# google-research/FirstOrderLp.jl

Measured on AMD Instinct MI355X. Metric: pdhg_iterations_per_sec, higher is better.
Workload: dtype f64; 1 GPU; random LP m=10000000 n=10000000 nnz=100000000 seed=12345 (BASELINE configs[4]), adaptive step, zero start, no restarts/rescaling; id=configs[4], m=10000000, n=10000000, nnz=100000000, parallelism=single GPU

## Files before the change

firstorderlp.jl_amd/csrc/abi_measure.hpp:

```cpp


int pdhg_profile_enable(pdhg_handle *h, int enable) {
  int rc0 = check_handle(h);
  if (rc0) return rc0;
  h->profile = enable != 0;
  if (enable) for (int k = 0; k < PDHG_K_COUNT; ++k) { h->prof_count[k] = 0; h->prof_ms[k] = 0.0; }
  return 0;
}

int pdhg_profile_read(pdhg_handle *h, int kernel_id, int64_t *launches, double *total_ms) {
  if (!h || kernel_id < 0 || kernel_id >= PDHG_K_COUNT) return fail(-1, "bad kernel id");
  *launches = h->prof_count[kernel_id];
  *total_ms = h->prof_ms[kernel_id];
  return 0;
}

int64_t pdhg_kernel_algorithmic_bytes(pdhg_handle *h, int kernel_id) {
  if (!h) return -1;
  const int64_t m = h->m, n = h->n, nnz = h->nnz, cn = h->cn;
  const bool group = h->grp != nullptr;
  switch (kernel_id) {
    case PDHG_K_PRIMAL: return 8 * (7 + (h->lazy_accept ? 2 : 0)) * cn;
    case PDHG_K_SPMV_DUAL:
      return nnz * 12 + (m + 1) * 4 + n * 8 + (3 + (h->lazy_accept ? 2 : 0)) * m * 8;
    case PDHG_K_SPMV_ATY:
      return nnz * 12 + (n + 1) * 4 + m * 8 + (group ? 1 : 4) * n * 8;
    case PDHG_K_FINAL: return 8 * (int64_t)(3 * h->At.slots() + h->A.slots());
    case PDHG_K_ACCEPT: return 8 * 3 * (cn + m);
    case PDHG_K_ALLGATHER: return group ? 8 * (h->n_alloc - h->grp->S) : 0;
    case PDHG_K_REDUCE_SCATTER: return group ? 8 * (h->n_alloc - h->grp->S) : 0;
    case PDHG_K_INTERACTION: return group ? 8 * 4 * cn : 0;
    default: return -1;
  }
}

namespace {
typedef double dbl2_t __attribute__((ext_vector_type(2)));
__global__ __launch_bounds__(TPB) void triad_kernel(int64_t len4, const dbl2_t *__restrict__ b,
                                                    const dbl2_t *__restrict__ c, double s,
                                                    dbl2_t *__restrict__ a) {
  const int64_t stride = (int64_t)gridDim.x * TPB;
  for (int64_t i = (int64_t)blockIdx.x * TPB + threadIdx.x; i < len4; i += stride) {
    const int64_t k = 2 * i;
    const dbl2_t b0 = __builtin_nontemporal_load(b + k), b1 = __builtin_nontemporal_load(b + k + 1);
    const dbl2_t c0 = __builtin_nontemporal_load(c + k), c1 = __builtin_nontemporal_load(c + k + 1);
// ... 288 lines not shown
    snprintf(b, sizeof b, ", \"sliced_jagged\": {\"window_rows\": %d, \"slices_per_wave\": %d, \"hub_threshold\": %d, \"hub_rows\": %lld, \"hub_nnz\": %lld, "
             "\"fill_narrow\": %.3f, \"fill_wide\": %.3f, \"ragged_share\": %.3f, \"grid\": %d}", SJ_SIGMA * J->G, J->G, J->max_len, (long long)hub, (long long)hub_nnz,
             J->fill_narrow, J->fill_wide, J->ragged, J->grid);
    out += b;
  }
  return out + "}";
}

int pdhg_layout_describe(pdhg_handle *h, char *buf, int cap) {
  if (!h) return fail(-1, "null handle");
  std::string out = "{\"A\": " + describe_matrix(h, h->A, MODE_DUAL, 0) + ", \"At\": " + describe_matrix(h, h->At, h->grp ? MODE_PLAIN : MODE_ATY, 1);
  if (h->has_q) out += ", \"Q\": " + describe_matrix(h, h->Q, MODE_PLAIN, 2) + ", \"Qt\": " + describe_matrix(h, h->Qt, MODE_PLAIN, 2);
  if (h->grp && !h->Achunk.empty()) {
    char b[256];
    snprintf(b, sizeof b, ", \"all_gather\": {\"chunks\": %d, \"mode\": \"%s\", \"columns_per_rank_and_chunk\": %lld, \"passes\": [",
             (int)h->Achunk.size(), (h->grp->ag_mode == 1 && h->grp->backend == COMM_RCCL) ? "overlapped with A_p xbar" : "passes behind one all-gather",
             (long long)h->grp->ag_sub);
    out += b;
    for (size_t c = 0; c < h->Achunk.size(); ++c)
      out += (c ? ", " : "") + describe_matrix(h, h->Achunk[c], c + 1 < h->Achunk.size() ? MODE_PLAIN : MODE_DUAL, 0);
    out += "]}";
  }
  const char *tv = getenv("PDHG_TUNE");
  out += std::string(", \"row_order\": \"") + (h->relaxed ? "relaxed" : "strict") + "\", \"timing_at_create\": " + ((tv && tv[0] == '0') ? "false" : "true") + "}";
  if (buf && cap > 0) {
    const size_t k = std::min(out.size(), (size_t)cap - 1);
    memcpy(buf, out.data(), k);
    buf[k] = 0;
  }
  return (int)out.size();
}

int pdhg_layout_info(pdhg_handle *h, int64_t info[16]) {
  if (!h) return fail(-1, "null handle");
  info[12] = (int64_t)h->A.slabs.size(); info[13] = (int64_t)h->At.slabs.size();
  info[14] = (coop_eligible(h) || h->coop_mode == 1) ? 2 : ((graph_eligible(h) || (h->graph_mode == 1 && !h->has_q)) ? 1 : 0);
  info[15] = ((h->A.tiled && h->A.var_tiles) || (!h->A.segs.empty() && h->A.segs.front().tiled && h->A.segs.front().var_tiles) ? 1 : 0) +
             ((h->At.tiled && h->At.var_tiles) || (!h->At.segs.empty() && h->At.segs.front().tiled && h->At.segs.front().var_tiles) ? 2 : 0) +
             (small_lp_eligible(h) ? 4 : 0) +
             (!h->grp && !h->has_q && !small_lp_eligible(h) && device_loop_for(h) && coop_eligible(h) ? 8 : 0) +
             (h->local_mode == 1 && h->local_launches > 0 ? 16 : 0);
  auto total = [](const CsrDev &D, auto f) { int64_t t = 0; if (D.segs.empty()) return (int64_t)f(D); for (const CsrDev &S : D.segs) t += f(S); return t; };
  auto first = [](const CsrDev &D) -> const CsrDev & { return D.segs.empty() ? D : D.segs.front(); };
  const CsrDev *Ms[2] = {&h->A, &h->At};
  for (int k = 0; k < 2; ++k) {
    const CsrDev &D = *Ms[k];
    info[4 * k + 0] = total(D, [](const CsrDev &S) { return S.nblk; });
// ... 21 lines not shown
```

firstorderlp.jl_amd/csrc/abi_rescale.hpp:

```cpp


static int row_grid(int rows) { return std::max(1, (rows + (TPB / WAVE) - 1) / (TPB / WAVE)); }

struct RescaleTmp {
  double *ev = nullptr, *dv = nullptr, *inv_e = nullptr, *inv_d = nullptr, *cum_e = nullptr, *cum_d = nullptr;
  double *tmp_e = nullptr, *tmp_d = nullptr;
};

extern "C++" {
template <int OP>
static void launch_row_op(pdhg_handle *h, const CsrDev &D, int cols, double pexp, const double *inv_scale, double *out) {
  if (!D.segs.empty()) {
    for (const CsrDev &S : D.segs) launch_row_op<OP>(h, S, cols, pexp, inv_scale ? inv_scale + S.row0 : inv_scale, out + S.row0);
    return;
  }
  hipLaunchKernelGGL(row_op_kernel<OP>, dim3(row_grid(D.rows)), dim3(TPB), 0, h->stream, D.view(), cols, pexp, inv_scale, out,
                     D.long_thr);
  if (D.nlong > 0) {
    hipLaunchKernelGGL(row_op_long_partial_kernel<OP>, dim3(D.nchunks), dim3(TPB), 0, h->stream, D.view(),
                       (const int *)D.chunk_row, (const int *)D.chunk_off, pexp, inv_scale, D.chunk_partial);
    hipLaunchKernelGGL(row_op_long_final_kernel<OP>, dim3(D.long_grid), dim3(TPB), 0, h->stream, D.view(),
                       (const int *)D.long_row, (const int *)D.long_chunk_ptr, D.nlong,
                       (const double *)D.chunk_partial, cols, pexp, out);
  }
// ... 23 lines not shown
        hipLaunchKernelGGL(scale_csr_kernel, dim3(row_grid(D.rows)), dim3(TPB), 0, h->stream, D.rows, S.rowptr,
                           S.col, S.val, inv_e, inv_d, k, 0);
    auto refill = [&](const SjDev &J, const int *rowptr, const int *col, const double *val) {
      if (J.on() && J.nnz > 0)
        hipLaunchKernelGGL(sj_fill_kernel, dim3((J.nslices + TPB / WAVE - 1) / (TPB / WAVE)), dim3(TPB), 0, h->stream, J.nslices, (TPB / WAVE) * J.G,
                           (const unsigned *)J.meta, (const int *)J.slice_off, rowptr, col, val, J.col, J.val);
    };
    refill(D.sj, D.rowptr, D.col, D.val);
    for (const SlabDev &S : D.slabs) refill(S.sj, S.rowptr, S.col, S.val);
  };
  scale_one(h->A, t.inv_e, t.inv_d, 0);
  scale_one(h->At, t.inv_e, t.inv_d, 1);
  if (!h->Achunk.empty() && h->grp) {
    DistGroup &g = *h->grp;
    int rc2 = launch_chunk_pack(g, t.inv_d, h->xchunk, 0, g.world, h->n, h->stream);
    if (rc2) return rc2;
    const int64_t W = (int64_t)g.world * g.ag_sub;
    for (size_t c = 0; c < h->Achunk.size(); ++c) scale_one(h->Achunk[c], t.inv_e, h->xchunk + (int64_t)c * W, 0);
  }
  if (h->has_q) {
    scale_one(h->Q, t.inv_d, t.inv_d, 0);
    scale_one(h->Qt, t.inv_d, t.inv_d, 1);
  }
  hipLaunchKernelGGL(resc_apply_vectors_kernel, dim3(h->ew_grid_nm), dim3(TPB), 0, h->stream, n, m, t.dv, t.ev,
                     h->c, h->lb, h->ub, h->b, t.cum_d, t.cum_e);
  HIP_TRY(hipGetLastError());
  if (h->bat) return batch_scale_members(h, t.dv, t.ev);
  return 0;
}

int pdhg_rescale(pdhg_handle *h0, int l_inf_ruiz_iterations, int l2_norm_rescaling,
                 int use_pock_chambolle, double pock_chambolle_alpha,
                 double *constraint_rescaling_out, double *variable_rescaling_out) {
  int rc = check_handle(h0, true, true);
  if (rc) return rc;
  if (h0->owner) return fail(-1, "pdhg_rescale: a batch member shares its batch's matrix: rescale the batch handle");
  if (use_pock_chambolle && !(pock_chambolle_alpha >= 0.0 && pock_chambolle_alpha <= 2.0))
    return fail(-1, "pock_chambolle_alpha must be in [0, 2]");
  const Shards L = shards_of(h0);
  if ((rc = flush_pending(L))) return rc;
  bump_version(L);
  for (int i = 0; i < L.count; ++i) L.p[i]->matrix_version += 1;
  std::vector<RescaleTmp> T((size_t)L.count);
  auto cleanup = [&]() {
    for (int i = 0; i < L.count; ++i) {
      (void)hipSetDevice(L.p[i]->device);
// ... 135 lines not shown
```

firstorderlp.jl_amd/csrc/common.hpp:

```cpp
#pragma once

namespace {

constexpr int TPB = 256;
constexpr int WAVE = 64;
constexpr int BLOCK_NNZ = 2048;
constexpr int UNROLL = BLOCK_NNZ / TPB;
#ifndef PDHG_MAX_ROWS_PER_BLOCK
#define PDHG_MAX_ROWS_PER_BLOCK (4 * TPB)
#endif
constexpr int MAX_ROWS_PER_BLOCK = PDHG_MAX_ROWS_PER_BLOCK;
inline const char *dev_env(const char *name) {
  static const bool on = [] { const char *e = getenv("PDHG_DEV"); return e && e[0] == '1'; }();
  return on ? getenv(name) : nullptr;
}
constexpr int LONG_CHUNK = BLOCK_NNZ;
inline int long_row_threshold_from_env() {
  const char *e = dev_env("PDHG_LONG_THR");
  const int v = e ? atoi(e) : BLOCK_NNZ;
  return v < 16 ? 16 : (v > BLOCK_NNZ ? BLOCK_NNZ : v);
}
constexpr int NUM_XCD = 8;
constexpr int EW_MAX_BLOCKS = 256 * 8;
inline int ew_grid(int64_t len) {
  return (int)std::max<int64_t>(1, std::min<int64_t>((len + TPB - 1) / TPB, EW_MAX_BLOCKS));
}
constexpr int FINAL_TPB = 1024;
constexpr int TW_WPB = 8;
constexpr int TW_MAX_ROWS = 1272;
constexpr unsigned TW_PAD = 0xFFFFFFFFu;
#ifndef TWD_U
#define TWD_U 4
#endif
constexpr int TW_U = TWD_U;

thread_local std::string g_last_error;

int fail(int code, const std::string &msg) {
  g_last_error = msg;
  return code;
}

int fail_hip(hipError_t e, const char *what) {
  g_last_error = std::string(what) + ": " + hipGetErrorString(e);
  return (int)e > 0 ? (int)e : 999;
}

#define HIP_TRY(expr)                                                        \
  do {                                                                       \
    hipError_t _e = (expr);                                                  \
    if (_e != hipSuccess) {                                                  \
      g_last_error = std::string(#expr) + ": " + hipGetErrorString(_e);      \
      return (int)_e > 0 ? (int)_e : 999;                                    \
    }                                                                        \
  } while (0)

struct RoctxApi {
// ... 176 lines not shown
```

firstorderlp.jl_amd/csrc/host_shards.hpp:

```cpp


template <typename Src, typename Dst>
int gather_cols_device(const Shards &L, Src src, Dst dst) {
  if (!L.g) {
    pdhg_handle *s = L.p[0];
    if (src(s) != dst(s))
      HIP_TRY(hipMemcpyAsync(dst(s), src(s), sizeof(double) * (size_t)s->n, hipMemcpyDeviceToDevice, s->stream));
    return 0;
  }
  FOR_SHARDS(L, s) {
    if (src(s) != dst(s) && s->cn > 0)
      HIP_TRY(hipMemcpyAsync(dst(s) + s->clo, src(s) + s->clo, sizeof(double) * (size_t)s->cn,
                             hipMemcpyDeviceToDevice, s->stream));
  }
  return dist_all_gather(*L.g, dst, L.g->S);
}

template <typename Src>
int cols_to_host(const Shards &L, Src src, double *host) {
  if (!L.g || L.g->all_local()) {
    FOR_SHARDS(L, s) {
      if (s->cn > 0)
        HIP_TRY(hipMemcpyAsync(host + s->clo, src(s) + s->clo, sizeof(double) * (size_t)s->cn, hipMemcpyDeviceToHost, s->stream));
    }
// ... 428 lines not shown
    if (len > 0) { HIP_TRY(hipMemcpy(*dst, src, sizeof(double) * (size_t)len, hipMemcpyHostToDevice)); HIP_TRY(hipStreamSynchronize(nullptr)); }
    return 0;
  };
  CK(up(&h->c, c, n)); CK(up(&h->b, b, m)); CK(up(&h->lb, lb, n)); CK(up(&h->ub, ub, n));
  CK(alloc_zero(&h->x, n_alloc)); CK(alloc_zero(&h->x_next, n_alloc)); CK(alloc_zero(&h->xbar, n_alloc));
  CK(alloc_zero(&h->y, m)); CK(alloc_zero(&h->y_next, m));
  CK(alloc_zero(&h->aty, n_alloc + 1)); CK(alloc_zero(&h->aty_next, n_alloc + 1));
  CK(alloc_zero(&h->sum_x, n)); CK(alloc_zero(&h->sum_y, m));
  CK(alloc_zero(&h->tmp_n, n_alloc)); CK(alloc_zero(&h->tmp_m, m));
  h->ew_grid_n = ew_grid(n); h->ew_grid_m = ew_grid(m); h->ew_grid_nm = ew_grid(std::max(n, m));
  h->pAt_stride = std::max(h->At.slots(), h->ew_grid_n);
  CK(alloc_zero(&h->pA, 2 * (int64_t)std::max(h->A.slots(), 1)));
  CK(alloc_zero(&h->pAt, 6 * (int64_t)std::max(h->pAt_stride, 1)));
  CK(alloc_zero(&h->pQ, 2 * (int64_t)h->ew_grid_n));
  CK(alloc_zero(&h->scal_dev, SCAL_MAX));
#undef CK
  hipError_t e = hipHostMalloc((void **)&h->scal_host, sizeof(double) * SCAL_MAX * DIST_MAX_WORLD, hipHostMallocDefault);
  if (e != hipSuccess) return fail((int)e, "hipHostMalloc failed");
  e = hipEventCreate(&h->ev0); if (e == hipSuccess) e = hipEventCreate(&h->ev1);
  if (e != hipSuccess) return fail((int)e, "hipEventCreate failed");
  return 0;
}

int create_shard(pdhg_handle **out, int64_t m, int64_t n, int64_t nnz,
                 const int64_t *colptr, const int64_t *rowval, const double *nzval,
                 int index_base, const double *c, const double *b, const double *lb,
                 const double *ub, int64_t num_equalities, int device_id, void *stream, int64_t n_alloc, int64_t seg_cap) {
  *out = nullptr;
  if (index_base != 0 && index_base != 1) return fail(-1, "index_base must be 0 or 1");
  if (num_equalities < 0 || num_equalities > m) return fail(-1, "num_equalities out of range");
  if (!colptr || !c || !lb || !ub || (m > 0 && !b) || (nnz > 0 && (!rowval || !nzval)))
    return fail(-1, "null input array");
  int ndev = 0;
  HIP_TRY(hipGetDeviceCount(&ndev));
  if (ndev <= 0) return fail(-3, "no HIP device visible");
  int dev = device_id;
  if (dev < 0) HIP_TRY(hipGetDevice(&dev));
  if (dev >= ndev) return fail(-1, "device_id out of range");
  HIP_TRY(hipSetDevice(dev));
  n_alloc = std::max(n_alloc, n);

  pdhg_handle *h = new pdhg_handle();
  h->self = h;
  h->device = dev;
  h->m = m; h->n = n; h->nnz = nnz; h->num_eq = num_equalities;
  h->cn = n; h->n_alloc = n_alloc; h->m_global = m;
  const char *env = getenv("PDHG_XCD_REMAP");
  h->remap = !(env && env[0] == '0');
  env = getenv("PDHG_ROW_ORDER");
  h->relaxed = !(env && !strcmp(env, "strict"));
  env = getenv("PDHG_LAZY_ACCEPT");
  h->lazy_accept = !(env && env[0] == '0');
  if (stream) { h->stream = (hipStream_t)stream; h->own_stream = false; }
  else {
    hipError_t e = hipStreamCreateWithFlags(&h->stream, hipStreamNonBlocking);
    if (e != hipSuccess) { delete h; return fail((int)e, "hipStreamCreate failed"); }
    h->own_stream = true;
  }
#define CK(expr) do { int _rc = (expr); if (_rc) { destroy_shard(h); return _rc; } } while (0)
  if (seg_cap > 0 && nnz > seg_cap) CK(build_segments(dev, h, m, n, nnz, colptr, rowval, nzval, index_base, seg_cap));
  else CK(build_layout_pair(dev, h->remap, h->relaxed, m, n, nnz, colptr, rowval, nzval, index_base, &h->A, &h->At));
  CK(alloc_shard_vectors(h, c, b, lb, ub));
  CK(tune_tiled_variant(h, h->A, h->xbar, h->tmp_m));
  CK(tune_tiled_variant(h, h->At, h->y, h->tmp_n));
#undef CK
  HIP_TRY(hipDeviceSynchronize());
  *out = h;
  return 0;
}

int trial_timeline(pdhg_handle *h, double out[14]) {
  if (!h->coop_trace || h->coop_grid <= 0) return 1;
  std::vector<unsigned long long> t((size_t)8 * h->coop_grid);
  if (hipMemcpy(t.data(), h->coop_trace, sizeof(unsigned long long) * t.size(), hipMemcpyDeviceToHost) != hipSuccess) return 1;
  unsigned long long t0 = ~0ull;
  for (int w = 0; w < h->coop_grid; ++w) t0 = std::min(t0, t[(size_t)w * 8]);
  for (int k = 0; k < 5; ++k) {
    double sum = 0, mx = 0, last_end = 0;
    for (int w = 0; w < h->coop_grid; ++w) {
      const double d = 0.01 * (double)(t[(size_t)w * 8 + k + 1] - t[(size_t)w * 8 + k]);
      sum += d; mx = std::max(mx, d);
      last_end = std::max(last_end, 0.01 * (double)(t[(size_t)w * 8 + k + 1] - t0));
    }
    out[k] = sum / h->coop_grid;
    out[5 + k] = mx;
// ... 24 lines not shown
      for (int k = 0; k < 5; ++k)
        fprintf(stderr, "    %-38s mean %6.2f us, max %6.2f us; last workgroup out at %6.2f us\n", names[k], t[k], t[5 + k], h->timeline_last_out[k]);
      if (t[11] > 0) fprintf(stderr, "    barrier 3: global phase complete at %6.2f us; decision known to the last workgroup at %6.2f us (multi-step kernel, last trial)\n",
                             t[11], t[12]);
      else fprintf(stderr, "    second-stage reduction published at %6.2f us\n", t[12]);
    }
  }
  if (!h->owner) { free_csr_dev(h->A); free_csr_dev(h->At); }
  free_csr_dev(h->Q); free_csr_dev(h->Qt);
  for (CsrDev &D : h->Achunk) free_csr_dev(D);
  if (h->chunk_carry) (void)hipFree(h->chunk_carry);
  if (h->xchunk) (void)hipFree(h->xchunk);
  for (hipEvent_t ev : h->ev_ag) if (ev) (void)hipEventDestroy(ev);
  if (h->ev_xbar) (void)hipEventDestroy(h->ev_xbar);
  double *bufs[] = {h->c, h->b, h->lb, h->ub, h->x, h->x_next, h->xbar, h->y, h->y_next,
                    h->aty, h->aty_next, h->sum_x, h->sum_y, h->qx, h->tmp_n, h->tmp_n2,
                    h->tmp_m, h->pA, h->pAt, h->pQ, h->scal_dev, h->scal_all, h->dn_buf, h->dm_buf,
                    h->E, h->Dv, h->c_o, h->b_o, h->lb_o,
                    h->ub_o, h->x_r, h->y_r, h->px_avg, h->py_avg, h->ev_ax, h->ev_aty, h->tr_g,
                    h->tr_dir, h->tr_thr, h->ev_partials, h->ev_cax[0], h->ev_cax[1], h->ev_cax[2],
                    h->ev_caty[0], h->ev_caty[1], h->ev_caty[2], h->ev_cqx[0], h->ev_cqx[1], h->ev_cqx[2],
                    h->ev_qx, h->ev_xg};
  for (double *p : bufs) if (p) (void)hipFree(p);
  graph_destroy(h->tgraph[0]); graph_destroy(h->tgraph[1]);
  if (h->comm_stream) { (void)hipStreamSynchronize(h->comm_stream); (void)hipStreamDestroy(h->comm_stream); }
  for (hipEvent_t ev : h->ev_part) if (ev) (void)hipEventDestroy(ev);
  if (h->ev_comm) (void)hipEventDestroy(h->ev_comm);
  if (h->seq_dev) (void)hipFree(h->seq_dev);
  if (h->gsync) (void)hipFree(h->gsync);
  if (h->tr_sync) (void)hipFree(h->tr_sync);
  if (h->lsync) (void)hipFree(h->lsync);
  if (h->tr_partials) (void)hipFree(h->tr_partials);
  if (h->trb_scratch) (void)hipFree(h->trb_scratch);
  if (h->trb_partials) (void)hipFree(h->trb_partials);
  if (h->coop_trace) (void)hipFree(h->coop_trace);
  if (h->res_host) (void)hipHostFree((void *)h->res_host);
  if (h->scal_host) (void)hipHostFree(h->scal_host);
  if (h->ev_host) (void)hipHostFree(h->ev_host);
  if (h->steps_ctl) (void)hipFree(h->steps_ctl);
  if (h->steps_pow_dev) (void)hipFree(h->steps_pow_dev);
  if (h->steps_pow_host) (void)hipHostFree(h->steps_pow_host);
  if (h->steps_res) (void)hipHostFree(h->steps_res);
  if (h->ev0) (void)hipEventDestroy(h->ev0);
  if (h->ev1) (void)hipEventDestroy(h->ev1);
  if (h->own_stream && h->stream) (void)hipStreamDestroy(h->stream);
  delete h;
// ... 166 lines not shown
```

firstorderlp.jl_amd/csrc/host_trial_graph_build.hpp:

```cpp

bool graph_eligible(pdhg_handle *h) {
  if (h->graph_mode < 0) {
    const char *ev = getenv("PDHG_GRAPH");
    const bool tiled_ok = dev_env("PDHG_GRAPH_TILED") != nullptr;
    bool on = !h->grp && !h->has_q && h->n > 0 && h->A.segs.empty() && h->At.segs.empty() && (tiled_ok || (!h->A.tiled && !h->At.tiled));
    if (ev) on = on && ev[0] != '0';
    h->graph_mode = on ? 1 : 0;
  }
  return h->graph_mode == 1 && !h->has_q && !h->profile;
}

void graph_destroy(pdhg_handle::TrialGraph &G) {
  if (G.exec) (void)hipGraphExecDestroy(G.exec);
  if (G.graph) (void)hipGraphDestroy(G.graph);
  G = pdhg_handle::TrialGraph();
}

struct GraphArgs {
  pdhg_handle *h;
  int n;
  dim3 primal_grid;
  EpiArgs dual_epi;
  GraphArgs(pdhg_handle *h_, double sigma) : h(h_), n((int)h_->n), primal_grid(ew_grid((h_->n + 1) / 2)) {
    dual_epi = EpiArgs{};
// ... 149 lines not shown
        HIP_TRY(graph_set_kernel(G.exec, G.n_dual, (const void *)spmv_stream_pipe_kernel<MODE_DUAL, true, 0>, dim3(S.pipe_grid), dim3(TPB),
                                 S.view(A.rows), (const double *)h->xbar, (const int4 *)S.ext, S.nblk, S.per_xcd, rm, rx, S.grid, le));
      else
        HIP_TRY(graph_set_kernel(G.exec, G.n_dual, (const void *)spmv_stream_kernel<MODE_DUAL, true, 0>, dim3(S.grid), dim3(TPB),
                                 S.view(A.rows), (const double *)h->xbar, (const int2 *)S.blks, (const int4 *)S.ext, S.nblk, S.per_xcd, rm, rx | 2, le));
    } else if (A.sj.on()) {
      HIP_TRY(graph_set_kernel(G.exec, G.n_dual, sj_kernel_fn<MODE_DUAL, false, 0>(A.sj), dim3(A.sj.grid), dim3(TPB),
                               sj_view(A.sj, rx), (const double *)h->xbar, rm, A.grid, dual_epi));
    } else if (A.pipe_grid > 0) {
      HIP_TRY(graph_set_kernel(G.exec, G.n_dual, (const void *)spmv_stream_pipe_kernel<MODE_DUAL, false, 0>, dim3(A.pipe_grid), dim3(TPB),
                               A.view(), (const double *)h->xbar, (const int4 *)A.ext, A.nblk, A.per_xcd, rm, rx, A.grid, dual_epi));
    } else {
      HIP_TRY(graph_set_kernel(G.exec, G.n_dual, (const void *)spmv_stream_kernel<MODE_DUAL, false, 0>, dim3(A.grid), dim3(TPB),
                               A.view(), (const double *)h->xbar, (const int2 *)A.blks, (const int4 *)A.ext, A.nblk, A.per_xcd, rm, rx, dual_epi));
    }
  }
  if (G.n_dual_long)
    HIP_TRY(graph_set_kernel(G.exec, G.n_dual_long, (const void *)spmv_long_final_kernel<MODE_DUAL>,
                             dim3(A.long_grid), dim3(TPB), (const int *)A.long_row, (const int *)A.long_chunk_ptr,
                             A.nlong, (const double *)A.chunk_partial, dual_epi, A.grid));
  return 0;
}

int graph_build(pdhg_handle *h, pdhg_handle::TrialGraph &G, double tau, double theta, double sigma) {
  graph_destroy(G);
  int rcw = ensure_result_word(h);
  if (rcw) return rcw;
  HIP_TRY(hipGraphCreate(&G.graph, 0));
  GraphArgs a(h, sigma);
  const double *nullq = nullptr;
  HIP_TRY(graph_add_kernel(G.graph, &G.n_primal, {}, (const void *)primal_kernel<false, true>, a.primal_grid, dim3(TPB),
                           a.n, (const double *)h->x, (const double *)h->c, (const double *)h->aty, nullq,
                           (const double *)h->lb, (const double *)h->ub, tau, theta, h->x_next, h->xbar,
                           h->pend_w, h->pend_x ? h->sum_x : (double *)nullptr));
  std::vector<hipGraphNode_t> dual_done, aty_done;
  {
    int rc = graph_add_spmv<MODE_DUAL, 0>(h, G.graph, h->A, h->xbar, a.dual_epi, {G.n_primal}, dual_done, &G.n_dual, &G.n_dual_long);
    if (rc) return rc;
  }
  if (dual_done.empty()) dual_done.push_back(G.n_primal);
  const CsrDev &A = h->A;
  const CsrDev &T = h->At;
  EpiArgs te{};
  te.x = h->x; te.x_next = h->x_next; te.aty = h->aty; te.aty_next = h->aty_next;
  te.partials = h->pAt; te.stride = h->pAt_stride; te.lo_offset = 3 * h->pAt_stride;
  {
    int rc = graph_add_spmv<MODE_ATY, 1>(h, G.graph, T, h->y_next, te, dual_done, aty_done, nullptr, nullptr);
    if (rc) return rc;
  }
  if (aty_done.empty()) aty_done = dual_done;
  FinalSpec sp{};
  sp.ptr[0] = h->pAt;                       sp.count[0] = T.slots();
  sp.ptr[1] = h->pAt + h->pAt_stride;       sp.count[1] = T.slots();
  sp.ptr[2] = h->pA;                        sp.count[2] = A.slots();
  sp.ptr[3] = h->pAt + 2 * h->pAt_stride;   sp.count[3] = T.slots();
  sp.ptr[4] = h->pQ;                        sp.count[4] = 0;
  for (int q : {0, 1, 3}) sp.ptr_lo[q] = sp.ptr[q] + 3 * h->pAt_stride;
// ... 6 lines not shown
  HIP_TRY(hipGraphInstantiate(&G.exec, G.graph, nullptr, nullptr, 0));
  G.x = h->x; G.y = h->y; G.aty = h->aty;
  G.tau = tau; G.theta = theta; G.sigma = sigma;
  G.add_x = h->pend_x; G.add_wx = h->pend_w;
  G.add_y = h->pend_y; G.add_wy = h->pend_w;
  return 0;
}

int graph_trial(pdhg_handle *h, double step_size, double primal_weight, double theta, double out[5]) {
  const double tau = step_size / primal_weight, sigma = primal_weight * step_size;
  pdhg_handle::TrialGraph *G = nullptr;
  for (int k = 0; k < 2; ++k)
    if (h->tgraph[k].exec && h->tgraph[k].x == h->x && h->tgraph[k].y == h->y && h->tgraph[k].aty == h->aty)
      G = &h->tgraph[k];
  if (!G) {
    G = !h->tgraph[0].exec ? &h->tgraph[0] : (!h->tgraph[1].exec ? &h->tgraph[1] : &h->tgraph[0]);
    int rc = graph_build(h, *G, tau, theta, sigma);
    if (rc) return rc;
  } else {
    const auto c0 = std::chrono::steady_clock::now();
    GraphArgs a(h, sigma);
    if (G->tau != tau || G->theta != theta || G->add_x != h->pend_x || (h->pend_x && G->add_wx != h->pend_w)) {
      const double *nullq = nullptr;
      HIP_TRY(graph_set_kernel(G->exec, G->n_primal, (const void *)primal_kernel<false, true>, a.primal_grid, dim3(TPB),
                               a.n, (const double *)h->x, (const double *)h->c, (const double *)h->aty, nullq,
                               (const double *)h->lb, (const double *)h->ub, tau, theta, h->x_next, h->xbar,
                               h->pend_w, h->pend_x ? h->sum_x : (double *)nullptr));
      G->tau = tau; G->theta = theta;
      G->add_x = h->pend_x; G->add_wx = h->pend_w;
    }
    if (G->sigma != sigma || G->add_y != h->pend_y || (h->pend_y && G->add_wy != h->pend_w)) {
      int rc = graph_set_dual(h, *G, a.dual_epi);
      if (rc) return rc;
      G->sigma = sigma;
      G->add_y = h->pend_y; G->add_wy = h->pend_w;
    }
    h->t_set += std::chrono::duration<double>(std::chrono::steady_clock::now() - c0).count();
  }
  h->seq_expected += 1;
  const auto c1 = std::chrono::steady_clock::now();
  HIP_TRY(hipGraphLaunch(G->exec, h->stream));
#ifdef PDHG_PROBE_GRAPH_TWICE
  HIP_TRY(hipGraphLaunch(G->exec, h->stream));
  h->seq_expected += 1;
#endif
  const auto c2 = std::chrono::steady_clock::now();
  h->t_launch += std::chrono::duration<double>(c2 - c1).count();
  h->n_graph_trials += 1;
  h->pend_x = h->pend_y = false;
  int rcw = wait_result_word(h, out);
// ... 47 lines not shown
```

firstorderlp.jl_amd/csrc/pdhg_hip.hip:

```cpp
#include <hip/hip_runtime.h>
#include <dlfcn.h>

#include <algorithm>
#include <atomic>
#include <chrono>
#include <condition_variable>
#include <functional>
#include <cmath>
#include <cstdint>
#include <cstdio>
#include <cstdlib>
#include <cstring>
#include <string>
#include <mutex>
#include <thread>
#include <vector>

#include "pdhg_hip.h"

#include "common.hpp"
#include "spmv_kernels.hpp"
#include "sj_kernels.hpp"
#include "vector_kernels.hpp"
#include "eval_kernels.hpp"
// ... 3 lines not shown
#include "trial_kernel.hpp"
#include "small_lp_kernel.hpp"
#include "tr_coop_kernel.hpp"
#include "batch_kernels.hpp"

namespace { struct DistGroup; struct FleetState; }
struct BatchState;

struct pdhg_handle {
  int device = 0;
  hipStream_t stream = nullptr;
  bool own_stream = false;
  int64_t m = 0, n = 0, nnz = 0, num_eq = 0;
  bool remap = true;
  bool relaxed = true;

  CsrDev A;
  CsrDev At;
  bool has_q = false;
  CsrDev Q;
  CsrDev Qt;

  double *c = nullptr, *b = nullptr, *lb = nullptr, *ub = nullptr;
  double *x = nullptr, *x_next = nullptr, *xbar = nullptr;
  double *y = nullptr, *y_next = nullptr;
  double *aty = nullptr, *aty_next = nullptr;
  double *sum_x = nullptr, *sum_y = nullptr;
  double *qx = nullptr, *tmp_n = nullptr, *tmp_n2 = nullptr, *tmp_m = nullptr;
  int64_t sum_x_count = 0, sum_y_count = 0;
  bool pend_x = false, pend_y = false, lazy_accept = true;
  double pend_w = 0.0;
  double sum_x_weights = 0.0, sum_y_weights = 0.0;

  double *pA = nullptr;
  double *pAt = nullptr;
  double *pQ = nullptr;
  int pAt_stride = 0;
  int ew_grid_n = 1, ew_grid_m = 1, ew_grid_nm = 1;


  double *E = nullptr, *Dv = nullptr, *c_o = nullptr, *b_o = nullptr, *lb_o = nullptr, *ub_o = nullptr;
  double *x_r = nullptr, *y_r = nullptr;
  double *px_avg = nullptr, *py_avg = nullptr;
  double *ev_ax = nullptr, *ev_aty = nullptr;
  double *ev_cax[3] = {nullptr, nullptr, nullptr}, *ev_caty[3] = {nullptr, nullptr, nullptr};
  double *ev_cqx[3] = {nullptr, nullptr, nullptr}, *ev_qx = nullptr;
// ... 288 lines not shown
                       D.view(), xin, D.chunk_row, D.chunk_off, D.chunk_partial);
    hipLaunchKernelGGL(spmv_long_final_kernel<MODE_PLAIN>, dim3(D.long_grid), dim3(TPB), 0, h->stream,
                       D.long_row, D.long_chunk_ptr, D.nlong, D.chunk_partial, e, D.grid);
  }
  if (g1 > g0) {
    int rc = launch_tiled<MODE_PLAIN>(h, D, xin, e, g0, g1);
    if (rc) return rc;
  }
  HIP_TRY(hipGetLastError());
  return 0;
}

int launch_primal(pdhg_handle *h, double tau, double theta, bool write_xbar) {
  ProfScope ps(h, PDHG_K_PRIMAL);
  if (h->has_q) {
    EpiArgs e{};
    e.out = h->qx;
    int rc = launch_spmv<MODE_PLAIN, 2>(h, h->Q, h->x, e);
    if (rc) return rc;
  }
  const int n = (int)h->cn;
  const int64_t o = h->clo;
  const int grid = ew_grid((h->cn + 1) / 2);
#define PK(HQ, WX)                                                                           \
  hipLaunchKernelGGL((primal_kernel<HQ, WX>), dim3(grid), dim3(TPB), 0, h->stream, n,        \
                     h->x + o, h->c + o, h->aty + o, h->has_q ? h->qx + o : nullptr, h->lb + o, h->ub + o, tau, theta, \
                     h->x_next + o, h->xbar + o, h->pend_w, h->pend_x ? h->sum_x + o : nullptr)
  if (h->has_q) { if (write_xbar) PK(true, true); else PK(true, false); }
  else          { if (write_xbar) PK(false, true); else PK(false, false); }
#undef PK
  HIP_TRY(hipGetLastError());
  h->pend_x = false;
  return 0;
}

int launch_xbar(pdhg_handle *h, double theta) {
  const int64_t o = h->clo;
  hipLaunchKernelGGL(xbar_kernel, dim3(ew_grid(h->cn)), dim3(TPB), 0, h->stream, (int)h->cn, h->x + o, h->x_next + o,
                     theta, h->xbar + o);
  HIP_TRY(hipGetLastError());
  return 0;
}

int launch_dual(pdhg_handle *h, double sigma) {
  ProfScope ps(h, PDHG_K_SPMV_DUAL);
  EpiArgs e{};
  e.y = h->y; e.b = h->b; e.y_next = h->y_next; e.sigma = sigma; e.num_eq = (int)h->num_eq;
  e.partials = h->pA; e.stride = h->A.slots(); e.lo_offset = h->A.slots();
  if (h->pend_y) { e.sum_y = h->sum_y; e.avg_w = h->pend_w; }
  const int rc = launch_spmv<MODE_DUAL, 0>(h, h->A, h->xbar, e);
  if (!rc) h->pend_y = false;
  return rc;
// ... 234 lines not shown
```

firstorderlp.jl_amd/csrc/spmv_kernels.hpp:

```cpp
#pragma once

namespace {


struct CsrView {
  int rows;
  const int *rowptr;
  const int *col;
  const double *val;
};

enum { MODE_PLAIN = 0, MODE_DUAL = 1, MODE_ATY = 2 };

struct EpiArgs {
  double *out;
  const double *y;
  const double *b;
  double *y_next;
  double sigma;
  int num_eq;
  const double *x;
  const double *x_next;
  const double *aty;
  double *aty_next;
// ... 544 lines not shown
    for (int i = 0; i < U; ++i) {
      const int k = kbeg + i * WAVE + lane;
      const bool ok = k < kend;
      pp[i] = ok ? __builtin_nontemporal_load(pk + k) : TW_PAD;
      vv[i] = ok ? __builtin_nontemporal_load(tv + k) : 0.0;
    }
  };

  int kprev = live ? tp[0] : 0;
#pragma unroll
  for (int s = 0; s < D; ++s) {
    ks[s] = kprev;
    ke[s] = (live && s < ntiles) ? tp[s + 1] : kprev;
    tl[s] = (s < ntiles) ? stile[s] : 0;
    kprev = ke[s];
    load_set(p[s], v[s], ks[s], ke[s]);
  }
  ks[D] = ke[D] = kprev;
  tl[D] = 0;
#pragma unroll
  for (int i = 0; i < U; ++i) { p[D][i] = TW_PAD; v[D][i] = 0.0; }
  int ke_ahead = (live && D < ntiles) ? tp[D + 1] : kprev;

  for (int t0 = 0; t0 < ntiles; t0 += R) {
#pragma unroll
    for (int s = 0; s < R; ++s) {
      const int t = t0 + s;
      if (t < ntiles) {
        const int f = (s + D) % R;
        const double *xt = xin + (size_t)tl[s];
#pragma unroll
        for (int i = 0; i < U; ++i) xv[i] = (p[s][i] != TW_PAD) ? xt[p[s][i] & cmask] : 0.0;
        ks[f] = ke[(s + D - 1) % R];
        ke[f] = ke_ahead;
        tl[f] = (t + D < ntiles) ? stile[t + D] : 0;
        load_set(p[f], v[f], ks[f], ke[f]);
        ke_ahead = (live && t + D + 1 < ntiles) ? tp[t + D + 2] : ke_ahead;
#pragma unroll
        for (int i = 0; i < U; ++i) {
          if (ks[s] + i * WAVE < ke[s]) {
            if (CH == 1) tiled_chunk_scratch(acc, scratch, p[s][i], v[s][i], xv[i], tile_shift, lane);
            else if (CH == 3) tiled_chunk_scan(acc, p[s][i], v[s][i], xv[i], tile_shift, lane);
            else if (CH == 4) tiled_chunk_hybrid(acc, p[s][i], v[s][i], xv[i], tile_shift, lane);
            else if (CH == 2) tiled_chunk_relaxed(acc, p[s][i], v[s][i], xv[i], tile_shift, lane);
            else tiled_chunk(acc, p[s][i], v[s][i], xv[i], tile_shift, lane);
          }
        }
        for (int kb = ks[s] + U * WAVE; kb < ke[s]; kb += WAVE) {
          const int k = kb + lane;
          const bool ok = k < ke[s];
          const unsigned pp = ok ? __builtin_nontemporal_load(pk + k) : TW_PAD;
          const double vv = ok ? __builtin_nontemporal_load(tv + k) : 0.0;
          const double xx = ok ? xt[pp & cmask] : 0.0;
          if (CH == 1) tiled_chunk_scratch(acc, scratch, pp, vv, xx, tile_shift, lane);
          else if (CH == 3) tiled_chunk_scan(acc, pp, vv, xx, tile_shift, lane);
          else if (CH == 4) tiled_chunk_hybrid(acc, pp, vv, xx, tile_shift, lane);
          else if (CH == 2) tiled_chunk_relaxed(acc, pp, vv, xx, tile_shift, lane);
          else tiled_chunk(acc, pp, vv, xx, tile_shift, lane);
        }
        __syncthreads();
      }
    }
  }
  const int nrows = rr.y - rr.x;
  for (int r = lane; r < nrows; r += WAVE) row_epilogue<MODE>(e, rr.x + r, acc[r], acc3);
  constexpr int NQ = ModeNQ<MODE>::value;
  if (NQ > 0) {
    block_sum_dd<NQ, TW_THREADS>(acc3, red);
    if (threadIdx.x == 0 && wg_live) {
#pragma unroll
      for (int q = 0; q < NQ; ++q) {
        e.partials[q * e.stride + g] = acc3.hi[q];
        e.partials[e.lo_offset + q * e.stride + g] = acc3.lo[q];
      }
    }
  }
}

__device__ __forceinline__ void long_chunk_load(const CsrView &A, int r, int off, StreamRegs &g) {
  g.r0 = g.r1 = r;
  g.k0 = A.rowptr[r] + off;
  g.k1 = min(g.k0 + LONG_CHUNK, A.rowptr[r + 1]);
#pragma unroll
  for (int i = 0; i < UNROLL; ++i) {
    const int k = g.k0 + threadIdx.x + i * TPB;
    const bool ok = k < g.k1;
    g.cidx[i] = ok ? __builtin_nontemporal_load(A.col + k) : 0;
    g.v[i] = ok ? __builtin_nontemporal_load(A.val + k) : 0.0;
// ... 80 lines not shown
```

firstorderlp.jl_amd/csrc/vector_kernels.hpp:

```cpp
#pragma once

namespace {


template <bool HAS_Q, bool WRITE_XBAR>
__device__ __forceinline__ void primal_one(double x, double c, double aty,
                                           double qx, double lb, double ub,
                                           double tau, double theta, double &xn,
                                           double &xb) {
  const double q = HAS_Q ? qx : 0.0;
  const double t0 = q + c;
  const double g = t0 - aty;
  const double t1 = tau * g;
  double v = x - t1;
  v = jl_min(ub, jl_max(lb, v));
  xn = v;
  if (WRITE_XBAR) {
    const double d = v - x;
    const double t2 = theta * d;
    xb = v + t2;
  }
}

template <bool HAS_Q, bool WRITE_XBAR, bool COH = false>
__device__ __forceinline__ void primal_body(
    int n, const double *x, const double *c, const double *aty, const double *qx,
    const double *lb, const double *ub, double tau, double theta, double *x_next, double *xbar,
    double avg_w, double *sum_x, int bid, int nb) {
  const int npair = n >> 1;
  const int stride = nb * TPB;
  for (int p = bid * TPB + threadIdx.x; p < npair; p += stride) {
    const double2 xv = reinterpret_cast<const double2 *>(x)[p];
    if (sum_x) {
      double2 sv = reinterpret_cast<double2 *>(sum_x)[p];
      const double t0 = xv.x * avg_w, t1 = xv.y * avg_w;
      sv.x = sv.x + t0;
      sv.y = sv.y + t1;
      reinterpret_cast<double2 *>(sum_x)[p] = sv;
    }
    const double2 cv = reinterpret_cast<const double2 *>(c)[p];
    double2 av;
    if (COH) { av.x = ldc<true>(aty + 2 * p); av.y = ldc<true>(aty + 2 * p + 1); }
    else av = reinterpret_cast<const double2 *>(aty)[p];
    const double2 lv = reinterpret_cast<const double2 *>(lb)[p];
    const double2 uv = reinterpret_cast<const double2 *>(ub)[p];
    double2 qv = {0.0, 0.0};
    if (HAS_Q) qv = reinterpret_cast<const double2 *>(qx)[p];
    double2 xn, xb;
    primal_one<HAS_Q, WRITE_XBAR>(xv.x, cv.x, av.x, qv.x, lv.x, uv.x, tau, theta, xn.x, xb.x);
    primal_one<HAS_Q, WRITE_XBAR>(xv.y, cv.y, av.y, qv.y, lv.y, uv.y, tau, theta, xn.y, xb.y);
    {
      reinterpret_cast<double2 *>(x_next)[p] = xn;
      if (WRITE_XBAR) reinterpret_cast<double2 *>(xbar)[p] = xb;
    }
  }
  if ((n & 1) && bid == 0 && threadIdx.x == 0) {
    const int j = n - 1;
    double xn, xb;
    if (sum_x) {
      const double t = x[j] * avg_w;
      sum_x[j] = sum_x[j] + t;
    }
    primal_one<HAS_Q, WRITE_XBAR>(x[j], c[j], ldc<COH>(aty + j), HAS_Q ? qx[j] : 0.0, lb[j], ub[j], tau, theta, xn, xb);
    x_next[j] = xn;
    if (WRITE_XBAR) xbar[j] = xb;
  }
}

template <bool HAS_Q, bool WRITE_XBAR>
__global__ __launch_bounds__(TPB) void primal_kernel(
    int n, const double *__restrict__ x, const double *__restrict__ c,
    const double *__restrict__ aty, const double *__restrict__ qx,
    const double *__restrict__ lb, const double *__restrict__ ub, double tau,
    double theta, double *__restrict__ x_next, double *__restrict__ xbar,
    double avg_w, double *__restrict__ sum_x) {
  primal_body<HAS_Q, WRITE_XBAR>(n, x, c, aty, qx, lb, ub, tau, theta, x_next, xbar, avg_w, sum_x, blockIdx.x, gridDim.x);
}

__device__ __forceinline__ void xbar_body(int n, const double *x, const double *x_next, double theta, double *xbar,
                                          int bid, int nb) {
  const int stride = nb * TPB;
  for (int j = bid * TPB + threadIdx.x; j < n; j += stride) {
    const double v = x_next[j];
    const double d = v - x[j];
    const double t = theta * d;
    xbar[j] = v + t;
  }
}
__global__ __launch_bounds__(TPB) void xbar_kernel(int n, const double *__restrict__ x,
                                                   const double *__restrict__ x_next,
                                                   double theta, double *__restrict__ xbar) {
  xbar_body(n, x, x_next, theta, xbar, blockIdx.x, gridDim.x);
}

__device__ __forceinline__ void diff_body(int n, const double *a, const double *b, double *out, int bid, int nb) {
  const int stride = nb * TPB;
  for (int j = bid * TPB + threadIdx.x; j < n; j += stride) out[j] = a[j] - b[j];
}
__device__ __forceinline__ void diff_pairs_body(int n, const double *a, const double *b, double *out, int bid, int nb) {
// ... 192 lines not shown
```

Measured before the change: 596.5 iterations/s.

## Compress variable bounds into class indices and prefetch tiled SpMV epilogue operands

At handle creation the host groups the (lb, ub) pairs into at most 256 distinct classes. When that succeeds, the primal kernel reads one byte per variable plus a small table instead of two doubles, which cuts primal-step memory traffic. The classes are dropped on rescale, because rescaling changes the bounds. Separately, the tiled SpMV issues its epilogue operand loads in batches, the first batch before the last tiles finish, to hide epilogue latency. The prefetch adds register pressure and an explicit waitcnt.

```diff
diff --git a/firstorderlp.jl_amd/csrc/abi_measure.hpp b/firstorderlp.jl_amd/csrc/abi_measure.hpp
--- a/firstorderlp.jl_amd/csrc/abi_measure.hpp
+++ b/firstorderlp.jl_amd/csrc/abi_measure.hpp
@@ -20,7 +20,7 @@
   const int64_t m = h->m, n = h->n, nnz = h->nnz, cn = h->cn;
   const bool group = h->grp != nullptr;
   switch (kernel_id) {
-    case PDHG_K_PRIMAL: return 8 * (7 + (h->lazy_accept ? 2 : 0)) * cn;
+    case PDHG_K_PRIMAL: return 8 * (7 + (h->lazy_accept ? 2 : 0)) * cn - ((h->nclass > 0 && !(h->clo & 1)) ? 15 * cn : 0);
     case PDHG_K_SPMV_DUAL:
       return nnz * 12 + (m + 1) * 4 + n * 8 + (3 + (h->lazy_accept ? 2 : 0)) * m * 8;
     case PDHG_K_SPMV_ATY:
@@ -355,7 +355,8 @@
     out += "]}";
   }
   const char *tv = getenv("PDHG_TUNE");
-  out += std::string(", \"row_order\": \"") + (h->relaxed ? "relaxed" : "strict") + "\", \"timing_at_create\": " + ((tv && tv[0] == '0') ? "false" : "true") + "}";
+  out += std::string(", \"row_order\": \"") + (h->relaxed ? "relaxed" : "strict") + "\", \"timing_at_create\": " + ((tv && tv[0] == '0') ? "false" : "true") +
+         ", \"bound_classes\": " + std::to_string(h->nclass) + "}";
   if (buf && cap > 0) {
     const size_t k = std::min(out.size(), (size_t)cap - 1);
     memcpy(buf, out.data(), k);
diff --git a/firstorderlp.jl_amd/csrc/abi_rescale.hpp b/firstorderlp.jl_amd/csrc/abi_rescale.hpp
--- a/firstorderlp.jl_amd/csrc/abi_rescale.hpp
+++ b/firstorderlp.jl_amd/csrc/abi_rescale.hpp
@@ -69,6 +69,11 @@
     scale_one(h->Q, t.inv_d, t.inv_d, 0);
     scale_one(h->Qt, t.inv_d, t.inv_d, 1);
   }
+  if (h->nclass > 0) {
+    HIP_TRY(hipStreamSynchronize(h->stream));
+    drop_bound_classes(h);
+    graph_destroy(h->tgraph[0]); graph_destroy(h->tgraph[1]);
+  }
   hipLaunchKernelGGL(resc_apply_vectors_kernel, dim3(h->ew_grid_nm), dim3(TPB), 0, h->stream, n, m, t.dv, t.ev,
                      h->c, h->lb, h->ub, h->b, t.cum_d, t.cum_e);
   HIP_TRY(hipGetLastError());
diff --git a/firstorderlp.jl_amd/csrc/common.hpp b/firstorderlp.jl_amd/csrc/common.hpp
--- a/firstorderlp.jl_amd/csrc/common.hpp
+++ b/firstorderlp.jl_amd/csrc/common.hpp
@@ -33,6 +33,14 @@
 #define TWD_U 4
 #endif
 constexpr int TW_U = TWD_U;
+#ifndef TWD_EPI_BATCH
+#define TWD_EPI_BATCH 4
+#endif
+#ifndef TWD_EPI_AHEAD
+#define TWD_EPI_AHEAD 1
+#endif
+constexpr int TW_EPI_BATCH = TWD_EPI_BATCH;
+constexpr int TW_EPI_AHEAD = TWD_EPI_AHEAD;
 
 thread_local std::string g_last_error;
 
diff --git a/firstorderlp.jl_amd/csrc/host_shards.hpp b/firstorderlp.jl_amd/csrc/host_shards.hpp
--- a/firstorderlp.jl_amd/csrc/host_shards.hpp
+++ b/firstorderlp.jl_amd/csrc/host_shards.hpp
@@ -474,6 +474,47 @@
   return 0;
 }
 
+void drop_bound_classes(pdhg_handle *h) {
+  if (h->bcls) (void)hipFree(h->bcls);
+  if (h->btab) (void)hipFree(h->btab);
+  h->bcls = nullptr; h->btab = nullptr; h->nclass = 0;
+}
+static int classify_bounds(pdhg_handle *h, const double *lb, const double *ub) {
+  drop_bound_classes(h);
+  const char *ev = dev_env("PDHG_BOUND_CLASSES");
+  const int64_t n = h->n;
+  if ((ev && ev[0] == '0') || n <= 0) return 0;
+  constexpr int MAXC = 256, SLOTS = 1024;
+  uint64_t klo[MAXC], kub[MAXC];
+  int slot[SLOTS];
+  for (int &v : slot) v = -1;
+  std::vector<unsigned char> cls((size_t)n);
+  int nc = 0, last = -1;
+  for (int64_t j = 0; j < n; ++j) {
+    uint64_t a, b;
+    memcpy(&a, lb + j, 8); memcpy(&b, ub + j, 8);
+    if (last >= 0 && klo[last] == a && kub[last] == b) { cls[(size_t)j] = (unsigned char)last; continue; }
+    uint64_t hsh = (a * 0x9E3779B97F4A7C15ull) ^ ((b + 0x7F4A7C15ull) * 0xC2B2AE3D27D4EB4Full);
+    unsigned s = (unsigned)(hsh >> 54) & (SLOTS - 1);
+    while (slot[s] >= 0 && !(klo[slot[s]] == a && kub[slot[s]] == b)) s = (s + 1) & (SLOTS - 1);
+    if (slot[s] < 0) {
+      if (nc == MAXC) return 0;
+      klo[nc] = a; kub[nc] = b; slot[s] = nc++;
+    }
+    last = slot[s];
+    cls[(size_t)j] = (unsigned char)last;
+  }
+  double tab[2 * MAXC] = {};
+  for (int k = 0; k < nc; ++k) { memcpy(&tab[2 * k], &klo[k], 8); memcpy(&tab[2 * k + 1], &kub[k], 8); }
+  hipError_t e = hipMalloc((void **)&h->bcls, (size_t)n + 1);
+  if (e == hipSuccess) e = hipMalloc((void **)&h->btab, sizeof tab);
+  if (e == hipSuccess) e = hipMemcpy(h->bcls, cls.data(), (size_t)n, hipMemcpyHostToDevice);
+  if (e == hipSuccess) e = hipMemcpy(h->btab, tab, sizeof tab, hipMemcpyHostToDevice);
+  if (e != hipSuccess) { drop_bound_classes(h); return fail_hip(e, "bound classes"); }
+  h->nclass = nc;
+  return 0;
+}
+
 int create_shard(pdhg_handle **out, int64_t m, int64_t n, int64_t nnz,
                  const int64_t *colptr, const int64_t *rowval, const double *nzval,
                  int index_base, const double *c, const double *b, const double *lb,
@@ -513,6 +554,7 @@
   if (seg_cap > 0 && nnz > seg_cap) CK(build_segments(dev, h, m, n, nnz, colptr, rowval, nzval, index_base, seg_cap));
   else CK(build_layout_pair(dev, h->remap, h->relaxed, m, n, nnz, colptr, rowval, nzval, index_base, &h->A, &h->At));
   CK(alloc_shard_vectors(h, c, b, lb, ub));
+  CK(classify_bounds(h, lb, ub));
   CK(tune_tiled_variant(h, h->A, h->xbar, h->tmp_m));
   CK(tune_tiled_variant(h, h->At, h->y, h->tmp_n));
 #undef CK
@@ -583,6 +625,7 @@
                     h->ev_caty[0], h->ev_caty[1], h->ev_caty[2], h->ev_cqx[0], h->ev_cqx[1], h->ev_cqx[2],
                     h->ev_qx, h->ev_xg};
   for (double *p : bufs) if (p) (void)hipFree(p);
+  drop_bound_classes(h);
   graph_destroy(h->tgraph[0]); graph_destroy(h->tgraph[1]);
   if (h->comm_stream) { (void)hipStreamSynchronize(h->comm_stream); (void)hipStreamDestroy(h->comm_stream); }
   for (hipEvent_t ev : h->ev_part) if (ev) (void)hipEventDestroy(ev);
diff --git a/firstorderlp.jl_amd/csrc/host_trial_graph_build.hpp b/firstorderlp.jl_amd/csrc/host_trial_graph_build.hpp
--- a/firstorderlp.jl_amd/csrc/host_trial_graph_build.hpp
+++ b/firstorderlp.jl_amd/csrc/host_trial_graph_build.hpp
@@ -195,6 +195,10 @@
   return 0;
 }
 
+const void *graph_primal_fn(const pdhg_handle *h) {
+  return h->nclass > 0 ? (const void *)primal_kernel<false, true, true> : (const void *)primal_kernel<false, true, false>;
+}
+
 int graph_build(pdhg_handle *h, pdhg_handle::TrialGraph &G, double tau, double theta, double sigma) {
   graph_destroy(G);
   int rcw = ensure_result_word(h);
@@ -202,10 +206,11 @@
   HIP_TRY(hipGraphCreate(&G.graph, 0));
   GraphArgs a(h, sigma);
   const double *nullq = nullptr;
-  HIP_TRY(graph_add_kernel(G.graph, &G.n_primal, {}, (const void *)primal_kernel<false, true>, a.primal_grid, dim3(TPB),
+  HIP_TRY(graph_add_kernel(G.graph, &G.n_primal, {}, graph_primal_fn(h), a.primal_grid, dim3(TPB),
                            a.n, (const double *)h->x, (const double *)h->c, (const double *)h->aty, nullq,
                            (const double *)h->lb, (const double *)h->ub, tau, theta, h->x_next, h->xbar,
-                           h->pend_w, h->pend_x ? h->sum_x : (double *)nullptr));
+                           h->pend_w, h->pend_x ? h->sum_x : (double *)nullptr,
+                           (const unsigned char *)h->bcls, (const double2 *)h->btab));
   std::vector<hipGraphNode_t> dual_done, aty_done;
   {
     int rc = graph_add_spmv<MODE_DUAL, 0>(h, G.graph, h->A, h->xbar, a.dual_epi, {G.n_primal}, dual_done, &G.n_dual, &G.n_dual_long);
@@ -258,10 +263,11 @@
     GraphArgs a(h, sigma);
     if (G->tau != tau || G->theta != theta || G->add_x != h->pend_x || (h->pend_x && G->add_wx != h->pend_w)) {
       const double *nullq = nullptr;
-      HIP_TRY(graph_set_kernel(G->exec, G->n_primal, (const void *)primal_kernel<false, true>, a.primal_grid, dim3(TPB),
+      HIP_TRY(graph_set_kernel(G->exec, G->n_primal, graph_primal_fn(h), a.primal_grid, dim3(TPB),
                                a.n, (const double *)h->x, (const double *)h->c, (const double *)h->aty, nullq,
                                (const double *)h->lb, (const double *)h->ub, tau, theta, h->x_next, h->xbar,
-                               h->pend_w, h->pend_x ? h->sum_x : (double *)nullptr));
+                               h->pend_w, h->pend_x ? h->sum_x : (double *)nullptr,
+                               (const unsigned char *)h->bcls, (const double2 *)h->btab));
       G->tau = tau; G->theta = theta;
       G->add_x = h->pend_x; G->add_wx = h->pend_w;
     }
diff --git a/firstorderlp.jl_amd/csrc/pdhg_hip.hip b/firstorderlp.jl_amd/csrc/pdhg_hip.hip
--- a/firstorderlp.jl_amd/csrc/pdhg_hip.hip
+++ b/firstorderlp.jl_amd/csrc/pdhg_hip.hip
@@ -49,6 +49,9 @@
   CsrDev Qt;
 
   double *c = nullptr, *b = nullptr, *lb = nullptr, *ub = nullptr;
+  unsigned char *bcls = nullptr;
+  double2 *btab = nullptr;
+  int nclass = 0;
   double *x = nullptr, *x_next = nullptr, *xbar = nullptr;
   double *y = nullptr, *y_next = nullptr;
   double *aty = nullptr, *aty_next = nullptr;
@@ -383,12 +386,16 @@
   const int n = (int)h->cn;
   const int64_t o = h->clo;
   const int grid = ew_grid((h->cn + 1) / 2);
-#define PK(HQ, WX)                                                                           \
-  hipLaunchKernelGGL((primal_kernel<HQ, WX>), dim3(grid), dim3(TPB), 0, h->stream, n,        \
+  const bool cls = h->nclass > 0 && !(o & 1);
+#define PK(HQ, WX, CL)                                                                       \
+  hipLaunchKernelGGL((primal_kernel<HQ, WX, CL>), dim3(grid), dim3(TPB), 0, h->stream, n,    \
                      h->x + o, h->c + o, h->aty + o, h->has_q ? h->qx + o : nullptr, h->lb + o, h->ub + o, tau, theta, \
-                     h->x_next + o, h->xbar + o, h->pend_w, h->pend_x ? h->sum_x + o : nullptr)
-  if (h->has_q) { if (write_xbar) PK(true, true); else PK(true, false); }
-  else          { if (write_xbar) PK(false, true); else PK(false, false); }
+                     h->x_next + o, h->xbar + o, h->pend_w, h->pend_x ? h->sum_x + o : nullptr,                        \
+                     CL ? (const unsigned char *)h->bcls + o : nullptr, CL ? (const double2 *)h->btab : nullptr)
+#define PKC(HQ, WX) do { if (cls) PK(HQ, WX, true); else PK(HQ, WX, false); } while (0)
+  if (h->has_q) { if (write_xbar) PKC(true, true); else PKC(true, false); }
+  else          { if (write_xbar) PKC(false, true); else PKC(false, false); }
+#undef PKC
 #undef PK
   HIP_TRY(hipGetLastError());
   h->pend_x = false;
diff --git a/firstorderlp.jl_amd/csrc/spmv_kernels.hpp b/firstorderlp.jl_amd/csrc/spmv_kernels.hpp
--- a/firstorderlp.jl_amd/csrc/spmv_kernels.hpp
+++ b/firstorderlp.jl_amd/csrc/spmv_kernels.hpp
@@ -590,6 +590,21 @@
   for (int i = 0; i < U; ++i) { p[D][i] = TW_PAD; v[D][i] = 0.0; }
   int ke_ahead = (live && D < ntiles) ? tp[D + 1] : kprev;
 
+  const int nrows = rr.y - rr.x;
+  auto epi_request = [&](EpiOps(&o)[TW_EPI_BATCH], int rb) {
+#pragma unroll
+    for (int j = 0; j < TW_EPI_BATCH; ++j) {
+      const int u = rr.x + rb + j * WAVE;
+      EpiArgs eu = e;
+      eu.y += u; eu.b += u; eu.x += u; eu.x_next += u; eu.aty += u;
+      if (e.sum_y) eu.sum_y += u;
+      if (rb + j * WAVE + lane < nrows) o[j] = epi_load<MODE>(eu, lane);
+    }
+  };
+  EpiOps pre[TW_EPI_BATCH];
+  const int t_pre = max(ntiles - TW_EPI_AHEAD, 0);
+  if (MODE != MODE_PLAIN && TW_EPI_AHEAD > 0 && ntiles == 0) epi_request(pre, 0);
+
   for (int t0 = 0; t0 < ntiles; t0 += R) {
 #pragma unroll
     for (int s = 0; s < R; ++s) {
@@ -599,6 +614,7 @@
         const double *xt = xin + (size_t)tl[s];
 #pragma unroll
         for (int i = 0; i < U; ++i) xv[i] = (p[s][i] != TW_PAD) ? xt[p[s][i] & cmask] : 0.0;
+        if (MODE != MODE_PLAIN && TW_EPI_AHEAD > 0 && t == t_pre) epi_request(pre, 0);
         ks[f] = ke[(s + D - 1) % R];
         ke[f] = ke_ahead;
         tl[f] = (t + D < ntiles) ? stile[t + D] : 0;
@@ -630,8 +646,26 @@
       }
     }
   }
-  const int nrows = rr.y - rr.x;
-  for (int r = lane; r < nrows; r += WAVE) row_epilogue<MODE>(e, rr.x + r, acc[r], acc3);
+  if (MODE == MODE_PLAIN) {
+    for (int r = lane; r < nrows; r += WAVE) row_epilogue<MODE>(e, rr.x + r, acc[r], acc3);
+  } else {
+    for (int rb = 0; rb < nrows; rb += TW_EPI_BATCH * WAVE) {
+      const int r0 = rb + lane;
+      EpiOps o[TW_EPI_BATCH];
+      if (TW_EPI_AHEAD > 0 && rb == 0) {
+#pragma unroll
+        for (int j = 0; j < TW_EPI_BATCH; ++j) o[j] = pre[j];
+      } else {
+        __builtin_amdgcn_s_waitcnt(0x0F70);
+        epi_request(o, rb);
+      }
+#pragma unroll
+      for (int j = 0; j < TW_EPI_BATCH; ++j) {
+        const int r = r0 + j * WAVE;
+        if (r < nrows) epi_apply<MODE>(e, rr.x + r, acc[r], o[j], acc3);
+      }
+    }
+  }
   constexpr int NQ = ModeNQ<MODE>::value;
   if (NQ > 0) {
     block_sum_dd<NQ, TW_THREADS>(acc3, red);
diff --git a/firstorderlp.jl_amd/csrc/vector_kernels.hpp b/firstorderlp.jl_amd/csrc/vector_kernels.hpp
--- a/firstorderlp.jl_amd/csrc/vector_kernels.hpp
+++ b/firstorderlp.jl_amd/csrc/vector_kernels.hpp
@@ -22,11 +22,11 @@
   }
 }
 
-template <bool HAS_Q, bool WRITE_XBAR, bool COH = false>
+template <bool HAS_Q, bool WRITE_XBAR, bool COH = false, bool CLS = false>
 __device__ __forceinline__ void primal_body(
     int n, const double *x, const double *c, const double *aty, const double *qx,
     const double *lb, const double *ub, double tau, double theta, double *x_next, double *xbar,
-    double avg_w, double *sum_x, int bid, int nb) {
+    double avg_w, double *sum_x, int bid, int nb, const unsigned char *cls = nullptr, const double2 *tab = nullptr) {
   const int npair = n >> 1;
   const int stride = nb * TPB;
   for (int p = bid * TPB + threadIdx.x; p < npair; p += stride) {
@@ -42,8 +42,16 @@
     double2 av;
     if (COH) { av.x = ldc<true>(aty + 2 * p); av.y = ldc<true>(aty + 2 * p + 1); }
     else av = reinterpret_cast<const double2 *>(aty)[p];
-    const double2 lv = reinterpret_cast<const double2 *>(lb)[p];
-    const double2 uv = reinterpret_cast<const double2 *>(ub)[p];
+    double2 lv, uv;
+    if (CLS) {
+      const unsigned k2 = reinterpret_cast<const unsigned short *>(cls)[p];
+      const double2 b0 = tab[k2 & 255u], b1 = tab[k2 >> 8];
+      lv.x = b0.x; uv.x = b0.y;
+      lv.y = b1.x; uv.y = b1.y;
+    } else {
+      lv = reinterpret_cast<const double2 *>(lb)[p];
+      uv = reinterpret_cast<const double2 *>(ub)[p];
+    }
     double2 qv = {0.0, 0.0};
     if (HAS_Q) qv = reinterpret_cast<const double2 *>(qx)[p];
     double2 xn, xb;
@@ -61,20 +69,22 @@
       const double t = x[j] * avg_w;
       sum_x[j] = sum_x[j] + t;
     }
-    primal_one<HAS_Q, WRITE_XBAR>(x[j], c[j], ldc<COH>(aty + j), HAS_Q ? qx[j] : 0.0, lb[j], ub[j], tau, theta, xn, xb);
+    const double lj = CLS ? tab[cls[j]].x : lb[j], uj = CLS ? tab[cls[j]].y : ub[j];
+    primal_one<HAS_Q, WRITE_XBAR>(x[j], c[j], ldc<COH>(aty + j), HAS_Q ? qx[j] : 0.0, lj, uj, tau, theta, xn, xb);
     x_next[j] = xn;
     if (WRITE_XBAR) xbar[j] = xb;
   }
 }
 
-template <bool HAS_Q, bool WRITE_XBAR>
+template <bool HAS_Q, bool WRITE_XBAR, bool CLS = false>
 __global__ __launch_bounds__(TPB) void primal_kernel(
     int n, const double *__restrict__ x, const double *__restrict__ c,
     const double *__restrict__ aty, const double *__restrict__ qx,
     const double *__restrict__ lb, const double *__restrict__ ub, double tau,
     double theta, double *__restrict__ x_next, double *__restrict__ xbar,
-    double avg_w, double *__restrict__ sum_x) {
-  primal_body<HAS_Q, WRITE_XBAR>(n, x, c, aty, qx, lb, ub, tau, theta, x_next, xbar, avg_w, sum_x, blockIdx.x, gridDim.x);
+    double avg_w, double *__restrict__ sum_x, const unsigned char *__restrict__ cls, const double2 *__restrict__ tab) {
+  primal_body<HAS_Q, WRITE_XBAR, false, CLS>(n, x, c, aty, qx, lb, ub, tau, theta, x_next, xbar, avg_w, sum_x, blockIdx.x,
+                                             gridDim.x, cls, tab);
 }
 
 __device__ __forceinline__ void xbar_body(int n, const double *x, const double *x_next, double theta, double *xbar,
```

New measurement: 564.2 iterations/s. -5.4%, worse.
